# ViTAE-Transformer/LeMeViT

Measured on AMD Instinct MI355X. Metric: images/sec LeMeViT-Base 224^2 bf16 fwd+bwd, higher is better.
Workload: dtype bf16; 1 GPU; lemevit_base 224x224 bf16-autocast train step (fwd+bwd+AdamW), batch 128/GPU, drop_path 0.1, random-init weights; global_batch=128, parallelism=dp1, launch=eager, weight-gradient GEMMs on a side stream

## Files before the change

### lemevit_amd/csrc/attn_mfma.hip

```cpp
#include <stdlib.h>
#include <atomic>
#include "common.h"
#include "attn_internal.h"

#ifndef LMV_XCD_REMAP
#define LMV_XCD_REMAP 1
#endif

namespace {

constexpr int D = 32;
typedef __attribute__((address_space(3))) bf16x4_t* lds4_t;

__device__ __forceinline__ int swz(int r, int c16) { return r * 64 + ((c16 ^ (((r >> 2) & 1) << 1)) << 4); }

template <int NTHREADS>
__device__ __forceinline__ void stage_rows2(unsigned char* sa, const bf16_t* ba, int64_t rsa, unsigned char* sb, const bf16_t* bb, int64_t rsb,
                                            int r0, int nrows, int L, int tid) {
  const int total = nrows * 4, last = max(L - 1, 0);
  for (int c0 = 0; c0 < total; c0 += NTHREADS * 4) {
    uint4 va[4], vb[4];
#pragma unroll
    for (int j = 0; j < 4; ++j) {
      const int c = min(c0 + j * NTHREADS + tid, total - 1), cc = c & 3;
// ... 132 lines not shown
        o0 = MFMA(vt0, ph, o0); o0 = MFMA(vt0, pl, o0);
        o1 = MFMA(vt1, ph, o1); o1 = MFMA(vt1, pl, o1);
      }
    }
    if (q < a.Lq) {
      const float inv = 1.f / l;
      o0 *= inv; o1 *= inv;
      store8(ob + (int64_t)q * a.o_rs, g, o0, o1);
      if (a.lse && g == 0) a.lse[((int64_t)b * a.H + h) * a.Lq + q] = m * a.scale + __logf(l);
    }
  }
}

template <int NKT, int LK = 0, bool PV16 = false>
__global__ __launch_bounds__(256) void mfma_fwd_kernel(const AttnArgs a, int qt_per_block) {
  const int nb = gridDim.x, n = nb * a.H * a.B;
  const int L = LMV_XCD_REMAP ? xcd_contiguous((int)blockIdx.x + nb * ((int)blockIdx.y + a.H * (int)blockIdx.z), n) : (int)blockIdx.x + nb * ((int)blockIdx.y + a.H * (int)blockIdx.z);
  mfma_fwd_body<NKT, LK, PV16>(a, qt_per_block, L % nb, (L / nb) % a.H, L / (nb * a.H));
}

template <int NKT1, int LK1, int NKT2, int LK2>
__global__ __launch_bounds__(256) void mfma_fwd_pair_kernel(const AttnArgs a1, const AttnArgs a2, int per1, int per2, int nblk1) {
  const int n1 = nblk1 * a1.H * a1.B;
  int id = (int)blockIdx.x;
  if (id < n1 && LMV_XCD_REMAP) id = xcd_contiguous(id, n1);
  if (id < n1) { const int bx = id % nblk1, t = id / nblk1; mfma_fwd_body<NKT1, LK1, true>(a1, per1, bx, t % a1.H, t / a1.H); }
  else { const int t = id - n1; mfma_fwd_body<NKT2, LK2, true>(a2, per2, 0, t % a2.H, t / a2.H); }
}

template <int NKT>
__global__ __launch_bounds__(256) void mfma_bwd_dq_kernel(const AttnArgs a, float* __restrict__ delta, int qt_per_block) {
  __shared__ __attribute__((aligned(16))) unsigned char sK[NKT * 16 * 64], sV[NKT * 16 * 64];
  const int tid = threadIdx.x, lane = tid & 63, wave = tid >> 6, h = blockIdx.y, b = blockIdx.z;
  const bf16_t* qb = reinterpret_cast<const bf16_t*>(a.q) + b * a.q_bs + h * D;
  const bf16_t* gb = reinterpret_cast<const bf16_t*>(a.d_o) + b * a.o_bs + h * D;
  const bf16_t* ob = reinterpret_cast<const bf16_t*>(a.o) + b * a.o_bs + h * D;
  bf16_t* dqb = reinterpret_cast<bf16_t*>(a.dq) + b * a.q_bs + h * D;
  stage_rows2<256>(sK, reinterpret_cast<const bf16_t*>(a.k) + b * a.k_bs + h * D, a.k_rs, sV, reinterpret_cast<const bf16_t*>(a.v) + b * a.v_bs + h * D, a.v_rs, 0, NKT * 16, a.Lk, tid);
  __syncthreads();
  const int nqt = (a.Lq + 15) >> 4;
  const int qt_end = min(nqt, (int)(blockIdx.x + 1) * qt_per_block);
  const int g = lane >> 4;
  const int64_t bh = ((int64_t)b * a.H + h) * a.Lq;
  for (int qt = blockIdx.x * qt_per_block + wave; qt < qt_end; qt += 4) {
    const int q = qt * 16 + (lane & 15);
    const bool vq = q < a.Lq;
    const bf16x8_t qf = load_frag_global(qb, a.q_rs, q, a.Lq, lane);
    const bf16x8_t gf = load_frag_global(gb, a.o_rs, q, a.Lq, lane);
    const bf16x8_t of = load_frag_global(ob, a.o_rs, q, a.Lq, lane);
    const float lse = vq ? a.lse[bh + q] : 0.f;
    float dl = 0.f;
#pragma unroll
    for (int j = 0; j < 8; ++j) dl += (float)gf[j] * (float)of[j];
    dl = group_sum4(dl);
    if (vq && g == 0) delta[bh + q] = dl;
    f32x4_t dq0 = {0.f, 0.f, 0.f, 0.f}, dq1 = {0.f, 0.f, 0.f, 0.f};
#pragma unroll
    for (int kb2 = 0; kb2 < NKT / 2; ++kb2) {
      f32x4_t ds[2];
#pragma unroll
      for (int t = 0; t < 2; ++t) {
        const int kt = 2 * kb2 + t;
        const f32x4_t s = MFMA(frag_n(sK, kt * 16, lane), qf, (f32x4_t{0.f, 0.f, 0.f, 0.f}));
        const f32x4_t dp = MFMA(frag_n(sV, kt * 16, lane), gf, (f32x4_t{0.f, 0.f, 0.f, 0.f}));
#pragma unroll
        for (int r = 0; r < 4; ++r) {
          const bool ok = vq && (kt * 16 + g * 4 + r < a.Lk);
          const float p = ok ? __expf(s[r] * a.scale - lse) : 0.f;
          ds[t][r] = p * (dp[r] - dl) * a.scale;
        }
      }
      const bf16x8_t dsf = pack8(ds[0], ds[1]);
      dq0 = MFMA(frag_t(sK, kb2 * 32, kb2 * 32 + 16, 0, lane), dsf, dq0);
      dq1 = MFMA(frag_t(sK, kb2 * 32, kb2 * 32 + 16, 16, lane), dsf, dq1);
    }
    if (vq) {
      store8(dqb + (int64_t)q * a.q_rs, g, dq0, dq1);
    }
  }
}

constexpr int QR_MAX = 448;

template <int NKT, int KW, bool ATOMIC, bool FUSEDQ = false, int LK = 0, int QRM = QR_MAX>
__device__ __forceinline__ void mfma_bwd_dkv_body(const AttnArgs& a, const float* __restrict__ delta, float* __restrict__ acc_k,
                                                  float* __restrict__ acc_v, int q_per_block, const int bx, const int h, const int b) {
  constexpr int QW = 4 / KW;
  constexpr int TPW = (NKT + KW - 1) / KW;
  const int Lk = LK ? LK : a.Lk;
  static_assert(!FUSEDQ || (NKT == 2 && KW == 1), "the fused dQ path is written for two key tiles per wave");
  __shared__ __attribute__((aligned(16))) unsigned char sQG[2 * QRM * 64];
  __shared__ __attribute__((aligned(16))) float sL[QRM], sDl[QRM];
  __shared__ __attribute__((aligned(16))) unsigned char sKV[FUSEDQ ? 2 * 32 * 64 : 16];
  unsigned char* sQ = sQG;
  unsigned char* sG = sQG + QRM * 64;
  const int tid = threadIdx.x, lane = tid & 63, wave = tid >> 6;
  const int kw = wave % KW, qw = wave / KW, g = lane >> 4;
  const int q0 = bx * q_per_block, q1 = min(a.Lq, q0 + q_per_block);
  const int nrows = ((q1 - q0 + 31) >> 5) << 5;
  const int64_t bh = ((int64_t)b * a.H + h) * a.Lq;
  stage_rows2<256>(sQ, reinterpret_cast<const bf16_t*>(a.q) + b * a.q_bs + h * D, a.q_rs, sG, reinterpret_cast<const bf16_t*>(a.d_o) + b * a.o_bs + h * D, a.o_rs, q0, nrows, q1, tid);
  const bf16_t* kb = reinterpret_cast<const bf16_t*>(a.k) + b * a.k_bs + h * D;
  const bf16_t* vb = reinterpret_cast<const bf16_t*>(a.v) + b * a.v_bs + h * D;
  for (int i = tid; i < nrows; i += 256) {
    const bool ok = q0 + i < q1;
    sL[i] = ok ? a.lse[bh + q0 + i] : 1e30f;
    if constexpr (FUSEDQ) {
      float dl = 0.f;
      if (ok) {
        const bf16_t* gp = reinterpret_cast<const bf16_t*>(a.d_o) + b * a.o_bs + (int64_t)(q0 + i) * a.o_rs + h * D;
        const bf16_t* op = reinterpret_cast<const bf16_t*>(a.o) + b * a.o_bs + (int64_t)(q0 + i) * a.o_rs + h * D;
        uint4 rg[4], ro[4];
#pragma unroll
        for (int c = 0; c < 4; ++c) { rg[c] = *reinterpret_cast<const uint4*>(gp + c * 8); ro[c] = *reinterpret_cast<const uint4*>(op + c * 8); }
#pragma unroll
        for (int c = 0; c < 4; ++c) {
          float gv[8], ov[8];
          chunk_to_f<bf16_t>(rg[c], gv); chunk_to_f<bf16_t>(ro[c], ov);
#pragma unroll
          for (int j = 0; j < 8; ++j) dl += gv[j] * ov[j];
        }
      }
      sDl[i] = dl;
    } else {
      sDl[i] = ok ? delta[bh + q0 + i] : 0.f;
    }
  }
  if constexpr (FUSEDQ) stage_rows2<256>(sKV, kb, a.k_rs, sKV + 32 * 64, vb, a.v_rs, 0, 32, Lk, tid);
  bf16x8_t kf[TPW], vf[TPW];
  f32x4_t dk[TPW][2], dv[TPW][2];
#pragma unroll
  for (int i = 0; i < TPW; ++i) {
    const int kt = kw + i * KW;
    kf[i] = load_frag_global(kb, a.k_rs, kt * 16 + (lane & 15), (kt < NKT) ? Lk : 0, lane);
    vf[i] = load_frag_global(vb, a.v_rs, kt * 16 + (lane & 15), (kt < NKT) ? Lk : 0, lane);
#pragma unroll
    for (int dt = 0; dt < 2; ++dt) { dk[i][dt] = f32x4_t{0.f, 0.f, 0.f, 0.f}; dv[i][dt] = f32x4_t{0.f, 0.f, 0.f, 0.f}; }
  }
  __syncthreads();
  const bool vkey = true;
  for (int qb = qw; qb * 32 < nrows; qb += QW) {
    const int r0 = qb * 32;
    const bf16x8_t qn0 = frag_n(sQ, r0, lane), qn1 = frag_n(sQ, r0 + 16, lane);
    const bf16x8_t gn0 = frag_n(sG, r0, lane), gn1 = frag_n(sG, r0 + 16, lane);
    const bf16x8_t qt0 = frag_t(sQ, r0, r0 + 16, 0, lane), qt1 = frag_t(sQ, r0, r0 + 16, 16, lane);
    const bf16x8_t gt0 = frag_t(sG, r0, r0 + 16, 0, lane), gt1 = frag_t(sG, r0, r0 + 16, 16, lane);
    const float4 l0 = *reinterpret_cast<const float4*>(sL + r0 + g * 4), l1 = *reinterpret_cast<const float4*>(sL + r0 + 16 + g * 4);
    const float4 d0 = *reinterpret_cast<const float4*>(sDl + r0 + g * 4), d1 = *reinterpret_cast<const float4*>(sDl + r0 + 16 + g * 4);
    const float lse[8] = {l0.x, l0.y, l0.z, l0.w, l1.x, l1.y, l1.z, l1.w};
    const float dl[8] = {d0.x, d0.y, d0.z, d0.w, d1.x, d1.y, d1.z, d1.w};
    if constexpr (FUSEDQ) {
      bf16_t* dqb = reinterpret_cast<bf16_t*>(a.dq) + b * a.q_bs + h * D;
#pragma unroll
      for (int t = 0; t < 2; ++t) {
        const int qi = r0 + t * 16 + (lane & 15);
        const float lq = sL[qi], dq_ = sDl[qi];
        const bf16x8_t qn = t ? qn1 : qn0, gn = t ? gn1 : gn0;
        f32x4_t dsq[2];
#pragma unroll
        for (int kt = 0; kt < 2; ++kt) {
          if (LK && kt * 16 >= LK) { dsq[kt] = f32x4_t{0.f, 0.f, 0.f, 0.f}; continue; }
          const f32x4_t sv = MFMA(kf[kt], qn, (f32x4_t{0.f, 0.f, 0.f, 0.f}));
          const f32x4_t dp = MFMA(vf[kt], gn, (f32x4_t{0.f, 0.f, 0.f, 0.f}));
#pragma unroll
          for (int r = 0; r < 4; ++r) {
            const bool kin = (LK && kt * 16 + 16 <= LK) ? true : (kt * 16 + g * 4 + r < Lk);
            const float pq = kin ? __expf(sv[r] * a.scale - lq) : 0.f;
            dsq[kt][r] = pq * (dp[r] - dq_) * a.scale;
          }
        }
        const bf16x8_t dsf = pack8(dsq[0], dsq[1]);
// ... 124 lines not shown
    for (int dt = 0; dt < 2; ++dt) { dk[i][dt] = f32x4_t{0.f, 0.f, 0.f, 0.f}; dv[i][dt] = f32x4_t{0.f, 0.f, 0.f, 0.f}; }
  }
  __syncthreads();
  bf16_t* dqb = reinterpret_cast<bf16_t*>(a.dq) + b * a.q_bs + h * D;
  for (int r0 = 0; r0 < nrows; r0 += 32) {
    const bf16x8_t qn0 = frag_n(sQ, r0, lane), qn1 = frag_n(sQ, r0 + 16, lane);
    const bf16x8_t gn0 = frag_n(sG, r0, lane), gn1 = frag_n(sG, r0 + 16, lane);
    const bf16x8_t qt0 = frag_t(sQ, r0, r0 + 16, 0, lane), qt1 = frag_t(sQ, r0, r0 + 16, 16, lane);
    const bf16x8_t gt0 = frag_t(sG, r0, r0 + 16, 0, lane), gt1 = frag_t(sG, r0, r0 + 16, 16, lane);
    const float4 l0 = *reinterpret_cast<const float4*>(sL + r0 + g * 4), l1 = *reinterpret_cast<const float4*>(sL + r0 + 16 + g * 4);
    const float4 d0 = *reinterpret_cast<const float4*>(sDl + r0 + g * 4), d1 = *reinterpret_cast<const float4*>(sDl + r0 + 16 + g * 4);
    const float lse[8] = {l0.x, l0.y, l0.z, l0.w, l1.x, l1.y, l1.z, l1.w};
    const float dl[8] = {d0.x, d0.y, d0.z, d0.w, d1.x, d1.y, d1.z, d1.w};
#pragma unroll
    for (int i = 0; i < TPW; ++i) {
      const int kt = wave + i * 4;
      if (kt >= NKT || kt * 16 >= Lk) continue;
      const bool kvalid = kt * 16 + (lane & 15) < Lk;
      const f32x4_t s0 = MFMA(qn0, kf[i], (f32x4_t{0.f, 0.f, 0.f, 0.f})), s1 = MFMA(qn1, kf[i], (f32x4_t{0.f, 0.f, 0.f, 0.f}));
      const f32x4_t p0 = MFMA(gn0, vf[i], (f32x4_t{0.f, 0.f, 0.f, 0.f})), p1 = MFMA(gn1, vf[i], (f32x4_t{0.f, 0.f, 0.f, 0.f}));
      f32x4_t pr[2], ds[2];
#pragma unroll
      for (int r = 0; r < 4; ++r) {
        const float e0 = kvalid ? __expf(s0[r] * a.scale - lse[r]) : 0.f, e1 = kvalid ? __expf(s1[r] * a.scale - lse[4 + r]) : 0.f;
        pr[0][r] = e0; pr[1][r] = e1;
        ds[0][r] = e0 * (p0[r] - dl[r]) * a.scale; ds[1][r] = e1 * (p1[r] - dl[4 + r]) * a.scale;
      }
      const bf16x8_t pf = pack8(pr[0], pr[1]), dsf = pack8(ds[0], ds[1]);
      dv[i][0] = MFMA(gt0, pf, dv[i][0]); dv[i][1] = MFMA(gt1, pf, dv[i][1]);
      dk[i][0] = MFMA(qt0, dsf, dk[i][0]); dk[i][1] = MFMA(qt1, dsf, dk[i][1]);
      const uint4 w = __builtin_bit_cast(uint4, dsf);
      *reinterpret_cast<uint2*>(sT(wave, 0, i) + (lane & 15) * 32 + g * 8) = make_uint2(w.x, w.y);
      *reinterpret_cast<uint2*>(sT(wave, 1, i) + (lane & 15) * 32 + g * 8) = make_uint2(w.z, w.w);
    }
    f32x4_t dq[2][2];
#pragma unroll
    for (int t = 0; t < 2; ++t) { dq[t][0] = f32x4_t{0.f, 0.f, 0.f, 0.f}; dq[t][1] = f32x4_t{0.f, 0.f, 0.f, 0.f}; }
    {
      const int rr = (lane & 15) >> 2, qq = lane & 3;
#pragma unroll
      for (int pp = 0; pp < NP; ++pp) {
        const int kta = wave + (2 * pp) * 4, ktb = wave + (2 * pp + 1) * 4;
        if (kta >= NKT || kta * 16 >= Lk) continue;
        const bool has_b = 2 * pp + 1 < TPW && ktb < NKT && ktb * 16 < Lk;
        const int rowb = has_b ? ktb * 16 : kta * 16;
        const bf16x8_t ka = frag_t(sK, kta * 16, rowb, 0, lane), kb2 = frag_t(sK, kta * 16, rowb, 16, lane);
#pragma unroll
        for (int t = 0; t < 2; ++t) {
          const bf16x4_t lo = __builtin_amdgcn_ds_read_tr16_b64_v4bf16((lds4_t)(sT(wave, t, 2 * pp) + (g * 4 + rr) * 32 + qq * 8));
          bf16x4_t hi = {(__bf16)0.f, (__bf16)0.f, (__bf16)0.f, (__bf16)0.f};
          if (has_b) hi = __builtin_amdgcn_ds_read_tr16_b64_v4bf16((lds4_t)(sT(wave, t, 2 * pp + (2 * pp + 1 < TPW ? 1 : 0)) + (g * 4 + rr) * 32 + qq * 8));
          const bf16x8_t dst = __builtin_shufflevector(lo, hi, 0, 1, 2, 3, 4, 5, 6, 7);
          dq[t][0] = MFMA(ka, dst, dq[t][0]); dq[t][1] = MFMA(kb2, dst, dq[t][1]);
        }
      }
    }
#pragma unroll
    for (int t = 0; t < 2; ++t)
#pragma unroll
      for (int hh = 0; hh < 2; ++hh) *reinterpret_cast<f32x4_t*>(sRed(wave, t * 2 + hh) + lane * 4) = dq[t][hh];
    __syncthreads();
    if (wave < 2) {
      f32x4_t x0 = {0.f, 0.f, 0.f, 0.f}, x1 = {0.f, 0.f, 0.f, 0.f};
#pragma unroll
      for (int w = 0; w < 4; ++w) {
        x0 += *reinterpret_cast<const f32x4_t*>(sRed(w, wave * 2) + lane * 4);
        x1 += *reinterpret_cast<const f32x4_t*>(sRed(w, wave * 2 + 1) + lane * 4);
      }
      const int q = r0 + wave * 16 + (lane & 15);
      if (q < Lq) store8(dqb + (int64_t)q * a.q_rs, g, x0, x1);
    }
    __syncthreads();
  }
#pragma unroll
  for (int i = 0; i < TPW; ++i) {
    const int kt = wave + i * 4, key = kt * 16 + (lane & 15);
    if (kt >= NKT || key >= Lk) continue;
    store8(reinterpret_cast<bf16_t*>(a.dk) + b * a.k_bs + (int64_t)key * a.k_rs + h * D, g, dk[i][0], dk[i][1]);
    store8(reinterpret_cast<bf16_t*>(a.dv) + b * a.v_bs + (int64_t)key * a.v_rs + h * D, g, dv[i][0], dv[i][1]);
  }
}


template <int NKT, int LK = 0>
__device__ __forceinline__ void mfma_bwd_fused_body2(const AttnArgs& a, const int h, const int b) {
  constexpr int TPW = (NKT + 3) / 4;
  constexpr int NPAIR = (NKT + 1) / 2;
  constexpr int NQ = NKT * 16;
  constexpr int TBUF = 4 * 2 * TPW * 512;
  __shared__ __attribute__((aligned(16))) unsigned char sQ[NQ * 64], sG[NQ * 64];
  __shared__ __attribute__((aligned(16))) unsigned char sKT[(2 * TBUF > NQ * 64) ? 2 * TBUF : NQ * 64];
  __shared__ __attribute__((aligned(16))) float sL[NQ], sDl[NQ];
  auto sT = [&](int buf, int w, int t, int slot) -> unsigned char* { return &sKT[buf * TBUF + ((w * 2 + t) * TPW + slot) * 512]; };
  const int tid = threadIdx.x, lane = tid & 63, wave = __builtin_amdgcn_readfirstlane(tid >> 6);
  const int g = lane >> 4;
  const int Lk = LK ? LK : a.Lk, Lq = a.Lq;
  const int nrows = ((Lq + 31) >> 5) << 5;
  const int64_t bh = ((int64_t)b * a.H + h) * Lq;
  const bf16_t* kb = reinterpret_cast<const bf16_t*>(a.k) + b * a.k_bs + h * D;
  const bf16_t* vb = reinterpret_cast<const bf16_t*>(a.v) + b * a.v_bs + h * D;
  stage_rows2<256>(sQ, reinterpret_cast<const bf16_t*>(a.q) + b * a.q_bs + h * D, a.q_rs, sG, reinterpret_cast<const bf16_t*>(a.d_o) + b * a.o_bs + h * D, a.o_rs, 0, nrows, Lq, tid);
  stage_rows2<256>(sKT, kb, a.k_rs, sKT, kb, a.k_rs, 0, NKT * 16, Lk, tid);
  for (int i = tid; i < nrows; i += 256) {
    const bool ok = i < Lq;
    sL[i] = ok ? a.lse[bh + i] : 1e30f;
    float dl = 0.f;
    if (ok) {
      const bf16_t* gp = reinterpret_cast<const bf16_t*>(a.d_o) + b * a.o_bs + (int64_t)i * a.o_rs + h * D;
      const bf16_t* op = reinterpret_cast<const bf16_t*>(a.o) + b * a.o_bs + (int64_t)i * a.o_rs + h * D;
      uint4 rg[4], ro[4];
#pragma unroll
      for (int c = 0; c < 4; ++c) { rg[c] = *reinterpret_cast<const uint4*>(gp + c * 8); ro[c] = *reinterpret_cast<const uint4*>(op + c * 8); }
#pragma unroll
      for (int c = 0; c < 4; ++c) {
        float gv[8], ov[8];
        chunk_to_f<bf16_t>(rg[c], gv); chunk_to_f<bf16_t>(ro[c], ov);
#pragma unroll
        for (int j = 0; j < 8; ++j) dl += gv[j] * ov[j];
      }
    }
    sDl[i] = dl;
  }
  bf16x8_t kf[TPW], vf[TPW];
  f32x4_t dk[TPW][2], dv[TPW][2];
#pragma unroll
  for (int i = 0; i < TPW; ++i) {
    const int kt = wave + i * 4;
    kf[i] = load_frag_global(kb, a.k_rs, kt * 16 + (lane & 15), (kt < NKT) ? Lk : 0, lane);
    vf[i] = load_frag_global(vb, a.v_rs, kt * 16 + (lane & 15), (kt < NKT) ? Lk : 0, lane);
#pragma unroll
    for (int dt = 0; dt < 2; ++dt) { dk[i][dt] = f32x4_t{0.f, 0.f, 0.f, 0.f}; dv[i][dt] = f32x4_t{0.f, 0.f, 0.f, 0.f}; }
  }
  __syncthreads();
  const int qt_w = wave >> 1, dh = wave & 1;
  bf16x8_t ktf[NPAIR];
#pragma unroll
  for (int pp = 0; pp < NPAIR; ++pp) {
    const int rowb = (2 * pp + 1 < NKT) ? (2 * pp + 1) * 16 : 2 * pp * 16;
    ktf[pp] = frag_t(sKT, 2 * pp * 16, rowb, dh * 16, lane);
  }
  __syncthreads();
  bf16_t* dqb = reinterpret_cast<bf16_t*>(a.dq) + b * a.q_bs + h * D;
  int buf = 0;
  for (int r0 = 0; r0 < nrows; r0 += 32, buf ^= 1) {
    const bf16x8_t qn0 = frag_n(sQ, r0, lane), qn1 = frag_n(sQ, r0 + 16, lane);
    const bf16x8_t gn0 = frag_n(sG, r0, lane), gn1 = frag_n(sG, r0 + 16, lane);
    const bf16x8_t qt0 = frag_t(sQ, r0, r0 + 16, 0, lane), qt1 = frag_t(sQ, r0, r0 + 16, 16, lane);
    const bf16x8_t gt0 = frag_t(sG, r0, r0 + 16, 0, lane), gt1 = frag_t(sG, r0, r0 + 16, 16, lane);
    const float4 l0 = *reinterpret_cast<const float4*>(sL + r0 + g * 4), l1 = *reinterpret_cast<const float4*>(sL + r0 + 16 + g * 4);
    const float4 d0 = *reinterpret_cast<const float4*>(sDl + r0 + g * 4), d1 = *reinterpret_cast<const float4*>(sDl + r0 + 16 + g * 4);
    const float lse[8] = {l0.x, l0.y, l0.z, l0.w, l1.x, l1.y, l1.z, l1.w};
    const float dl[8] = {d0.x, d0.y, d0.z, d0.w, d1.x, d1.y, d1.z, d1.w};
#pragma unroll
    for (int i = 0; i < TPW; ++i) {
      const int kt = wave + i * 4;
      if (kt >= NKT || kt * 16 >= Lk) continue;
      const bool kvalid = kt * 16 + (lane & 15) < Lk;
      const f32x4_t s0 = MFMA(qn0, kf[i], (f32x4_t{0.f, 0.f, 0.f, 0.f})), s1 = MFMA(qn1, kf[i], (f32x4_t{0.f, 0.f, 0.f, 0.f}));
      const f32x4_t p0 = MFMA(gn0, vf[i], (f32x4_t{0.f, 0.f, 0.f, 0.f})), p1 = MFMA(gn1, vf[i], (f32x4_t{0.f, 0.f, 0.f, 0.f}));
      f32x4_t pr[2], ds[2];
#pragma unroll
      for (int r = 0; r < 4; ++r) {
        const float e0 = kvalid ? __expf(s0[r] * a.scale - lse[r]) : 0.f, e1 = kvalid ? __expf(s1[r] * a.scale - lse[4 + r]) : 0.f;
        pr[0][r] = e0; pr[1][r] = e1;
        ds[0][r] = e0 * (p0[r] - dl[r]) * a.scale; ds[1][r] = e1 * (p1[r] - dl[4 + r]) * a.scale;
      }
      const bf16x8_t pf = pack8(pr[0], pr[1]), dsf = pack8(ds[0], ds[1]);
      dv[i][0] = MFMA(gt0, pf, dv[i][0]); dv[i][1] = MFMA(gt1, pf, dv[i][1]);
      dk[i][0] = MFMA(qt0, dsf, dk[i][0]); dk[i][1] = MFMA(qt1, dsf, dk[i][1]);
      const uint4 w = __builtin_bit_cast(uint4, dsf);
      const int wsl = (g ^ ((lane >> 2) & 3)) * 8;
      *reinterpret_cast<uint2*>(sT(buf, wave, 0, i) + (lane & 15) * 32 + wsl) = make_uint2(w.x, w.y);
      *reinterpret_cast<uint2*>(sT(buf, wave, 1, i) + (lane & 15) * 32 + wsl) = make_uint2(w.z, w.w);
    }
    __syncthreads();
    {
      const int rr = (lane & 15) >> 2, qq = lane & 3;
      f32x4_t dq = {0.f, 0.f, 0.f, 0.f};
#pragma unroll
      for (int pp = 0; pp < NPAIR; ++pp) {
        const int kta = 2 * pp, ktb = 2 * pp + 1;
        if (kta * 16 >= Lk) continue;
        const bool has_b = ktb < NKT && ktb * 16 < Lk;
        const bf16x4_t lo = __builtin_amdgcn_ds_read_tr16_b64_v4bf16((lds4_t)(sT(buf, kta & 3, qt_w, kta >> 2) + (g * 4 + rr) * 32 + (qq ^ g) * 8));
        bf16x4_t hi = {(__bf16)0.f, (__bf16)0.f, (__bf16)0.f, (__bf16)0.f};
        if (has_b) hi = __builtin_amdgcn_ds_read_tr16_b64_v4bf16((lds4_t)(sT(buf, ktb & 3, qt_w, ktb >> 2) + (g * 4 + rr) * 32 + (qq ^ g) * 8));
        const bf16x8_t dst = __builtin_shufflevector(lo, hi, 0, 1, 2, 3, 4, 5, 6, 7);
        dq = MFMA(ktf[pp], dst, dq);
      }
      const int q = r0 + qt_w * 16 + (lane & 15);
      if (q < Lq) store4(dqb + (int64_t)q * a.q_rs + g * 8 + dh * 4, dq);
    }
  }
#pragma unroll
  for (int i = 0; i < TPW; ++i) {
    const int kt = wave + i * 4, key = kt * 16 + (lane & 15);
    if (kt >= NKT || key >= Lk) continue;
    store8(reinterpret_cast<bf16_t*>(a.dk) + b * a.k_bs + (int64_t)key * a.k_rs + h * D, g, dk[i][0], dk[i][1]);
    store8(reinterpret_cast<bf16_t*>(a.dv) + b * a.v_bs + (int64_t)key * a.v_rs + h * D, g, dv[i][0], dv[i][1]);
  }
}

template <int NKT, int LK = 0, int VER = 1>
__global__ __launch_bounds__(256, 2) void mfma_bwd_fused_kernel(const AttnArgs a) {
  const int n = a.H * a.B, id = (int)blockIdx.y + a.H * (int)blockIdx.z;
  const int L = LMV_XCD_REMAP ? xcd_contiguous(id, n) : id;
  if constexpr (VER == 2) mfma_bwd_fused_body2<NKT, LK>(a, L % a.H, L / a.H);
  else mfma_bwd_fused_body<NKT, LK>(a, L % a.H, L / a.H);
}

template <int NKT1, int LK1, int VER = 1>
__global__ __launch_bounds__(256, 2) void mfma_bwd_pair_kernel(const AttnArgs a1, const AttnArgs a2) {
  const int n1 = a1.H * a1.B;
  int id = (int)blockIdx.x;
  if (id < n1 && LMV_XCD_REMAP) id = xcd_contiguous(id, n1);
  if (id < n1) { if constexpr (VER == 2) mfma_bwd_fused_body2<NKT1, LK1>(a1, id % a1.H, id / a1.H); else mfma_bwd_fused_body<NKT1, LK1>(a1, id % a1.H, id / a1.H); }
  else mfma_bwd_dkv_body<2, 1, false, true, 16, 32>(a2, nullptr, nullptr, nullptr, 32, 0, (id - n1) % a2.H, (id - n1) / a2.H);
}

__global__ __launch_bounds__(256) void scatter_bf16_kernel(const float* __restrict__ acc, bf16_t* __restrict__ dst, int64_t bs, int64_t rs, int B, int H,
                                                          int L, int LP) {
  const unsigned idx = blockIdx.x * 256 + threadIdx.x, total = (unsigned)B * H * L * D;
  if (idx >= total) return;
  const unsigned d = idx % D, l = (idx / D) % L, h = (idx / (D * L)) % H, b = idx / (D * L * H);
  dst[b * bs + (int64_t)l * rs + h * D + d] = f2bf(acc[((((int64_t)b * H + h) * LP) + l) * D + d]);
}

__global__ __launch_bounds__(256) void scatter_sum_kernel(const float* __restrict__ acc0, const float* __restrict__ acc1, bf16_t* __restrict__ dst0,
                                                         bf16_t* __restrict__ dst1, int64_t bs0, int64_t rs0, int64_t bs1, int64_t rs1, int B, int H, int L,
                                                         int LP, int nslab) {
  const unsigned idx = blockIdx.x * 256 + threadIdx.x, per = (unsigned)B * H * L * (D / 4);
  if (idx >= 2 * per) return;
  const bool second = idx >= per;
  const unsigned i = second ? idx - per : idx;
  const unsigned d4 = i % (D / 4), l = (i / (D / 4)) % L, h = (i / ((D / 4) * L)) % H, b = i / ((D / 4) * L * H);
  const float* src = (second ? acc1 : acc0) + ((((int64_t)b * H + h) * LP) + l) * D + d4 * 4;
  const int64_t slab = (int64_t)B * H * LP * D;
  f32x4_t s = {0.f, 0.f, 0.f, 0.f};
  for (int k = 0; k < nslab; ++k) s += *reinterpret_cast<const f32x4_t*>(src + k * slab);
  bf16_t* dst = second ? dst1 + b * bs1 + (int64_t)l * rs1 + h * D + d4 * 4 : dst0 + b * bs0 + (int64_t)l * rs0 + h * D + d4 * 4;
  store4(dst, s);
}

constexpr int RKT = 8, RK = RKT * 16;
constexpr int RKT_B = 4, RKB = RKT_B * 16;

__global__ __launch_bounds__(256) void mfma_fwd_split_kernel(const AttnArgs a, float* __restrict__ part, int nsplit) {
  __shared__ __attribute__((aligned(16))) unsigned char sK[4 * RK * 64], sV[4 * RK * 64];
  const int tid = threadIdx.x, lane = tid & 63, wave = tid >> 6, g = lane >> 4;
  const int nbx = gridDim.x, Lid = LMV_XCD_REMAP ? xcd_contiguous((int)blockIdx.x + nbx * ((int)blockIdx.y + a.H * (int)blockIdx.z), nbx * a.H * a.B)
                                                 : (int)blockIdx.x + nbx * ((int)blockIdx.y + a.H * (int)blockIdx.z);
  const int bx = Lid % nbx, h = (Lid / nbx) % a.H, b = Lid / (nbx * a.H);
  const int split = bx * 4 + wave, k0 = split * RK;
  const bf16_t* kb = reinterpret_cast<const bf16_t*>(a.k) + b * a.k_bs + h * D;
  const bf16_t* vb = reinterpret_cast<const bf16_t*>(a.v) + b * a.v_bs + h * D;
  unsigned char* wK = sK + wave * RK * 64;
  unsigned char* wV = sV + wave * RK * 64;
  stage_rows2<64>(wK, kb, a.k_rs, wV, vb, a.v_rs, k0, RK, a.Lk, lane);
  asm volatile("s_waitcnt vmcnt(0) lgkmcnt(0)" ::: "memory");
  __builtin_amdgcn_wave_barrier();
  if (split >= nsplit) return;
  const int q = lane & 15;
  float* pp = part + ((((int64_t)b * a.H + h) * nsplit + split) * 16 + q) * (D + 2);
  if (k0 >= a.Lk) {
    if (g == 0) { pp[0] = -1e30f; pp[1] = 0.f; }
#pragma unroll
    for (int r = 0; r < 4; ++r) { pp[2 + g * 4 + r] = 0.f; pp[18 + g * 4 + r] = 0.f; }
    return;
  }
  const bf16x8_t qf = load_frag_global(reinterpret_cast<const bf16_t*>(a.q) + b * a.q_bs + h * D, a.q_rs, q, a.Lq, lane);
  f32x4_t s[RKT];
  float m = -1e30f;
#pragma unroll
  for (int kt = 0; kt < RKT; ++kt) {
    s[kt] = MFMA(frag_n(wK, kt * 16, lane), qf, (f32x4_t{0.f, 0.f, 0.f, 0.f}));
#pragma unroll
    for (int r = 0; r < 4; ++r) {
      s[kt][r] = (k0 + kt * 16 + g * 4 + r < a.Lk) ? s[kt][r] * a.scale : -1e30f;
      m = fmaxf(m, s[kt][r]);
    }
  }
  m = group_max4(m);
  float l = 0.f;
#pragma unroll
  for (int kt = 0; kt < RKT; ++kt)
#pragma unroll
    for (int r = 0; r < 4; ++r) { const float p = __expf(s[kt][r] - m); s[kt][r] = p; l += p; }
  l = group_sum4(l);
  f32x4_t o0 = {0.f, 0.f, 0.f, 0.f}, o1 = {0.f, 0.f, 0.f, 0.f};
#pragma unroll
  for (int kb2 = 0; kb2 < RKT / 2; ++kb2) {
    const bf16x8_t ph = pack8(s[2 * kb2], s[2 * kb2 + 1]);
    f32x4_t r0, r1;
#pragma unroll
    for (int r = 0; r < 4; ++r) { r0[r] = s[2 * kb2][r] - (float)ph[r]; r1[r] = s[2 * kb2 + 1][r] - (float)ph[4 + r]; }
    const bf16x8_t pl = pack8(r0, r1);
    const bf16x8_t vt0 = frag_t(wV, kb2 * 32, kb2 * 32 + 16, 0, lane), vt1 = frag_t(wV, kb2 * 32, kb2 * 32 + 16, 16, lane);
    o0 = MFMA(vt0, ph, o0); o0 = MFMA(vt0, pl, o0);
    o1 = MFMA(vt1, ph, o1); o1 = MFMA(vt1, pl, o1);
  }
// ... 580 lines not shown
  dkv_split(a, &nsplit, &qpb);
  return 2 * (size_t)nsplit * a.B * a.H * nkt_for(a.Lk) * 16 * D * sizeof(float);
}

int lmv_attn_mfma_fwd(const AttnArgs& a, hipStream_t st) {
  const int per = qt_per_block_for(a), nqt = (a.Lq + 15) / 16;
  dim3 grid((nqt + per - 1) / per, a.H, a.B), block(256);
  if (a.Lk == 196) hipLaunchKernelGGL((mfma_fwd_kernel<14, 196, true>), grid, block, 0, st, a, per);
  else if (a.Lk == 16) hipLaunchKernelGGL((mfma_fwd_kernel<2, 16, true>), grid, block, 0, st, a, per);
  else if (a.Lk == 49) hipLaunchKernelGGL((mfma_fwd_kernel<4, 49, true>), grid, block, 0, st, a, per);
  else
  switch (nkt_for(a.Lk)) {
    case 2: hipLaunchKernelGGL((mfma_fwd_kernel<2>), grid, block, 0, st, a, per); break;
    case 4: hipLaunchKernelGGL((mfma_fwd_kernel<4>), grid, block, 0, st, a, per); break;
    case 8: hipLaunchKernelGGL((mfma_fwd_kernel<8>), grid, block, 0, st, a, per); break;
    default: hipLaunchKernelGGL((mfma_fwd_kernel<14>), grid, block, 0, st, a, per); break;
  }
  LMV_CHECK_LAUNCH("attn_mfma_fwd");
  return LMV_OK;
}

int lmv_attn_mfma_bwd(const AttnArgs& a, float* delta, float* acc, hipStream_t st) {
  const int per = qt_per_block_for(a), nqt = (a.Lq + 15) / 16, nkt = nkt_for(a.Lk);
  if (nkt >= 4 && a.Lq > 16 && a.Lq <= nkt * 16) {
    dim3 grid(1, a.H, a.B), block(256);
    if (a.Lk == 196) hipLaunchKernelGGL((mfma_bwd_fused_kernel<14, 196, 2>), grid, block, 0, st, a);
    else if (a.Lk == 49) hipLaunchKernelGGL((mfma_bwd_fused_kernel<4, 49, 2>), grid, block, 0, st, a);
    else if (nkt == 4) hipLaunchKernelGGL((mfma_bwd_fused_kernel<4>), grid, block, 0, st, a);
    else if (nkt == 8) hipLaunchKernelGGL((mfma_bwd_fused_kernel<8>), grid, block, 0, st, a);
    else hipLaunchKernelGGL((mfma_bwd_fused_kernel<14>), grid, block, 0, st, a);
    LMV_CHECK_LAUNCH("attn_mfma_bwd_fused");
    return LMV_OK;
  }
  if (nkt == 14 && a.Lq > 16) {
    int nk, pr, lds;
    if (int rc = long_geometry(a, &nk, &pr, &lds)) return rc;
    hipLaunchKernelGGL(mfma_bwd_dq_long_kernel, dim3((nqt + pr - 1) / pr, a.H, a.B), dim3(256), lds, st, a, delta, pr, nk);
  } else if (nkt != 2) {
    dim3 grid((nqt + per - 1) / per, a.H, a.B), block(256);
    switch (nkt) {
      case 4: hipLaunchKernelGGL((mfma_bwd_dq_kernel<4>), grid, block, 0, st, a, delta, per); break;
      case 8: hipLaunchKernelGGL((mfma_bwd_dq_kernel<8>), grid, block, 0, st, a, delta, per); break;
      default: hipLaunchKernelGGL((mfma_bwd_dq_kernel<14>), grid, block, 0, st, a, delta, per); break;
    }
  }
  int nsplit, qpb;
  dkv_split(a, &nsplit, &qpb);
  dim3 grid(nsplit, a.H, a.B), block(256);
  const size_t acc_elems = (size_t)nsplit * a.B * a.H * nkt * 16 * D;
  float* acc_k = acc; float* acc_v = acc + acc_elems;
  if (nsplit > 1) {
#define DKV(N, K) hipLaunchKernelGGL((mfma_bwd_dkv_kernel<N, K, true>), grid, block, 0, st, a, delta, acc_k, acc_v, qpb)
    if (nkt == 2 && a.Lk == 16) hipLaunchKernelGGL((mfma_bwd_dkv_kernel<2, 1, true, true, 16>), grid, block, 0, st, a, delta, acc_k, acc_v, qpb);
    else if (nkt == 2) hipLaunchKernelGGL((mfma_bwd_dkv_kernel<2, 1, true, true>), grid, block, 0, st, a, delta, acc_k, acc_v, qpb);
    else
    switch (nkt) { case 4: DKV(4, 2); break; case 8: DKV(8, 4); break; default: DKV(14, 4); break; }
#undef DKV
    const unsigned n = 2u * (unsigned)a.B * a.H * a.Lk * (D / 4);
    hipLaunchKernelGGL(scatter_sum_kernel, dim3((n + 255) / 256), dim3(256), 0, st, (const float*)acc_k, (const float*)acc_v, (bf16_t*)a.dk, (bf16_t*)a.dv,
                       a.k_bs, a.k_rs, a.v_bs, a.v_rs, a.B, a.H, a.Lk, nkt * 16, nsplit);
  } else {
#define DKV(N, K) hipLaunchKernelGGL((mfma_bwd_dkv_kernel<N, K, false>), grid, block, 0, st, a, delta, acc_k, acc_v, qpb)
    if (nkt == 2 && a.Lk == 16) hipLaunchKernelGGL((mfma_bwd_dkv_kernel<2, 1, false, true, 16>), grid, block, 0, st, a, delta, acc_k, acc_v, qpb);
    else if (nkt == 2) hipLaunchKernelGGL((mfma_bwd_dkv_kernel<2, 1, false, true>), grid, block, 0, st, a, delta, acc_k, acc_v, qpb);
    else
    switch (nkt) { case 4: DKV(4, 2); break; case 8: DKV(8, 4); break; default: DKV(14, 4); break; }
#undef DKV
  }
  LMV_CHECK_LAUNCH("attn_mfma_bwd");
  return LMV_OK;
}

int lmv_attn_mfma_fwd_pair(const AttnArgs& a1, const AttnArgs& a2, hipStream_t st) {
  if (a1.B != a2.B || a1.H != a2.H || a2.Lk != 16 || a2.Lq != 16 || a1.Lq != a1.Lk || (a1.Lk != 196 && a1.Lk != 49)) return 0;
  const int per1 = qt_per_block_for(a1), nqt1 = (a1.Lq + 15) / 16, nblk1 = (nqt1 + per1 - 1) / per1;
  dim3 grid((nblk1 + 1) * a1.H * a1.B), block(256);
  if (a1.Lk == 196) hipLaunchKernelGGL((mfma_fwd_pair_kernel<14, 196, 2, 16>), grid, block, 0, st, a1, a2, per1, 1, nblk1);
  else hipLaunchKernelGGL((mfma_fwd_pair_kernel<4, 49, 2, 16>), grid, block, 0, st, a1, a2, per1, 1, nblk1);
  return 1;
}

int lmv_attn_mfma_bwd_pair(const AttnArgs& a1, const AttnArgs& a2, hipStream_t st) {
  if (a1.B != a2.B || a1.H != a2.H || a2.Lk != 16 || a2.Lq != 16 || a1.Lq != a1.Lk || (a1.Lk != 196 && a1.Lk != 49)) return 0;
  dim3 grid(2 * a1.H * a1.B), block(256);
  if (a1.Lk == 196) hipLaunchKernelGGL((mfma_bwd_pair_kernel<14, 196, 2>), grid, block, 0, st, a1, a2);
  else hipLaunchKernelGGL((mfma_bwd_pair_kernel<4, 49, 2>), grid, block, 0, st, a1, a2);
  return 1;
}
```

Measured before the change: 4278 images/sec.

## Use 8-wave fused attention backward for 196 tokens and per-image meta-token blocks

Result: no change. 4258 images/sec (median of 2 runs) (-0.5%).

```diff
diff --git a/lemevit_amd/csrc/attn_mfma.hip b/lemevit_amd/csrc/attn_mfma.hip
--- a/lemevit_amd/csrc/attn_mfma.hip
+++ b/lemevit_amd/csrc/attn_mfma.hip
@@ -238,11 +238,12 @@
 
 constexpr int QR_MAX = 448;
 
-template <int NKT, int KW, bool ATOMIC, bool FUSEDQ = false, int LK = 0, int QRM = QR_MAX>
+template <int NKT, int KW, bool ATOMIC, bool FUSEDQ = false, int LK = 0>
 __device__ __forceinline__ void mfma_bwd_dkv_body(const AttnArgs& a, const float* __restrict__ delta, float* __restrict__ acc_k,
                                                   float* __restrict__ acc_v, int q_per_block, const int bx, const int h, const int b) {
   constexpr int QW = 4 / KW;
   constexpr int TPW = (NKT + KW - 1) / KW;
+  constexpr int QRM = QR_MAX;
   const int Lk = LK ? LK : a.Lk;
   static_assert(!FUSEDQ || (NKT == 2 && KW == 1), "the fused dQ path is written for two key tiles per wave");
   __shared__ __attribute__((aligned(16))) unsigned char sQG[2 * QRM * 64];
@@ -533,16 +534,24 @@
 }
 
 
+template <int NKT>
+constexpr int bwd_body2_lds() {
+  constexpr int TBUF = 4 * 2 * ((NKT + 3) / 4) * 512, NQ = NKT * 16;
+  return 2 * NQ * 64 + ((2 * TBUF > NQ * 64) ? 2 * TBUF : NQ * 64) + 2 * NQ * 4;
+}
 template <int NKT, int LK = 0>
-__device__ __forceinline__ void mfma_bwd_fused_body2(const AttnArgs& a, const int h, const int b) {
+__device__ __forceinline__ void mfma_bwd_fused_body2(const AttnArgs& a, const int h, const int b, unsigned char* smem) {
   constexpr int TPW = (NKT + 3) / 4;
   constexpr int NPAIR = (NKT + 1) / 2;
   constexpr int NQ = NKT * 16;
   constexpr int TBUF = 4 * 2 * TPW * 512;
-  __shared__ __attribute__((aligned(16))) unsigned char sQ[NQ * 64], sG[NQ * 64];
-  __shared__ __attribute__((aligned(16))) unsigned char sKT[(2 * TBUF > NQ * 64) ? 2 * TBUF : NQ * 64];
-  __shared__ __attribute__((aligned(16))) float sL[NQ], sDl[NQ];
-  auto sT = [&](int buf, int w, int t, int slot) -> unsigned char* { return &sKT[buf * TBUF + ((w * 2 + t) * TPW + slot) * 512]; };
+  constexpr int KTSZ = (2 * TBUF > NQ * 64) ? 2 * TBUF : NQ * 64;
+  unsigned char* sQ = smem;
+  unsigned char* sG = smem + NQ * 64;
+  unsigned char* sKT = smem + 2 * NQ * 64;
+  float* sL = reinterpret_cast<float*>(sKT + KTSZ);
+  float* sDl = sL + NQ;
+  auto sT = [&](int buf, int w, int t, int slot) -> unsigned char* { return sKT + buf * TBUF + ((w * 2 + t) * TPW + slot) * 512; };
   const int tid = threadIdx.x, lane = tid & 63, wave = __builtin_amdgcn_readfirstlane(tid >> 6);
   const int g = lane >> 4;
   const int Lk = LK ? LK : a.Lk, Lq = a.Lq;
@@ -652,21 +661,236 @@
   }
 }
 
+template <int NKT>
+constexpr int bwd_body3_lds() { return 3 * NKT * 16 * 64 + 2 * (16 * 2 * 512) + 2 * NKT * 16 * 4; }
+template <int NKT, int LK>
+__device__ __forceinline__ void mfma_bwd_fused_body3(const AttnArgs& a, const int h, const int b, unsigned char* smem) {
+  constexpr int NW = 8, NT = NW * 64, TPW = 2;
+  constexpr int NPAIR = (NKT + 1) / 2;
+  constexpr int NQ = NKT * 16;
+  constexpr int TBUF = NW * TPW * 2 * 512;
+  static_assert(LK > 0 && NKT > NW && NKT <= NW * TPW && (NKT & 1) == 0, "written for 9 .. 16 key tiles with a compile-time key count");
+  unsigned char* sQ = smem;
+  unsigned char* sG = smem + NQ * 64;
+  unsigned char* sK = smem + 2 * NQ * 64;
+  unsigned char* sTB = smem + 3 * NQ * 64;
+  float* sL = reinterpret_cast<float*>(sTB + 2 * TBUF);
+  float* sDl = sL + NQ;
+  auto sT = [&](int buf, int kt, int t) -> unsigned char* { return sTB + buf * TBUF + (kt * 2 + t) * 512; };
+  const int tid = threadIdx.x, lane = tid & 63, wave = __builtin_amdgcn_readfirstlane(tid >> 6);
+  const int g = lane >> 4;
+  constexpr int Lk = LK;
+  const int Lq = a.Lq;
+  const int nrows = ((Lq + 31) >> 5) << 5;
+  const int64_t bh = ((int64_t)b * a.H + h) * Lq;
+  const bf16_t* kb = reinterpret_cast<const bf16_t*>(a.k) + b * a.k_bs + h * D;
+  const bf16_t* vb = reinterpret_cast<const bf16_t*>(a.v) + b * a.v_bs + h * D;
+  stage_rows2<NT>(sQ, reinterpret_cast<const bf16_t*>(a.q) + b * a.q_bs + h * D, a.q_rs, sG, reinterpret_cast<const bf16_t*>(a.d_o) + b * a.o_bs + h * D, a.o_rs, 0, nrows, Lq, tid);
+  stage_rows2<NT>(sK, kb, a.k_rs, sK, kb, a.k_rs, 0, NKT * 16, Lk, tid);
+  for (int i = tid; i < nrows; i += NT) {
+    const bool ok = i < Lq;
+    sL[i] = ok ? a.lse[bh + i] : 1e30f;
+    float dl = 0.f;
+    if (ok) {
+      const bf16_t* gp = reinterpret_cast<const bf16_t*>(a.d_o) + b * a.o_bs + (int64_t)i * a.o_rs + h * D;
+      const bf16_t* op = reinterpret_cast<const bf16_t*>(a.o) + b * a.o_bs + (int64_t)i * a.o_rs + h * D;
+      uint4 rg[4], ro[4];
+#pragma unroll
+      for (int c = 0; c < 4; ++c) { rg[c] = *reinterpret_cast<const uint4*>(gp + c * 8); ro[c] = *reinterpret_cast<const uint4*>(op + c * 8); }
+#pragma unroll
+      for (int c = 0; c < 4; ++c) {
+        float gv[8], ov[8];
+        chunk_to_f<bf16_t>(rg[c], gv); chunk_to_f<bf16_t>(ro[c], ov);
+#pragma unroll
+        for (int j = 0; j < 8; ++j) dl += gv[j] * ov[j];
+      }
+    }
+    sDl[i] = dl;
+  }
+  bf16x8_t kf[TPW], vf[TPW];
+  f32x4_t dk[TPW][2], dv[TPW][2];
+#pragma unroll
+  for (int i = 0; i < TPW; ++i) {
+    const int kt = wave + i * NW;
+    kf[i] = load_frag_global(kb, a.k_rs, kt * 16 + (lane & 15), (kt < NKT) ? Lk : 0, lane);
+    vf[i] = load_frag_global(vb, a.v_rs, kt * 16 + (lane & 15), (kt < NKT) ? Lk : 0, lane);
+#pragma unroll
+    for (int dt = 0; dt < 2; ++dt) { dk[i][dt] = f32x4_t{0.f, 0.f, 0.f, 0.f}; dv[i][dt] = f32x4_t{0.f, 0.f, 0.f, 0.f}; }
+  }
+  __syncthreads();
+  bf16_t* dqb = reinterpret_cast<bf16_t*>(a.dq) + b * a.q_bs + h * D;
+  int buf = 0;
+  for (int r0 = 0; r0 < nrows; r0 += 32, buf ^= 1) {
+    {
+        const float4 l0 = *reinterpret_cast<const float4*>(sL + r0 + g * 4), l1 = *reinterpret_cast<const float4*>(sL + r0 + 16 + g * 4);
+        const float4 d0 = *reinterpret_cast<const float4*>(sDl + r0 + g * 4), d1 = *reinterpret_cast<const float4*>(sDl + r0 + 16 + g * 4);
+        const float lse[8] = {l0.x, l0.y, l0.z, l0.w, l1.x, l1.y, l1.z, l1.w};
+        const float dl[8] = {d0.x, d0.y, d0.z, d0.w, d1.x, d1.y, d1.z, d1.w};
+#pragma unroll
+      for (int i = 0; i < TPW; ++i) {
+        const int kt = wave + i * NW;
+        if (kt >= NKT || kt * 16 >= Lk) continue;
+        const bf16x8_t qn0 = frag_n(sQ, r0, lane), qn1 = frag_n(sQ, r0 + 16, lane);
+        const bf16x8_t gn0 = frag_n(sG, r0, lane), gn1 = frag_n(sG, r0 + 16, lane);
+        const bool kvalid = kt * 16 + (lane & 15) < Lk;
+        const f32x4_t s0 = MFMA(qn0, kf[i], (f32x4_t{0.f, 0.f, 0.f, 0.f})), s1 = MFMA(qn1, kf[i], (f32x4_t{0.f, 0.f, 0.f, 0.f}));
+        const f32x4_t p0 = MFMA(gn0, vf[i], (f32x4_t{0.f, 0.f, 0.f, 0.f})), p1 = MFMA(gn1, vf[i], (f32x4_t{0.f, 0.f, 0.f, 0.f}));
+        f32x4_t pr[2], ds[2];
+#pragma unroll
+        for (int r = 0; r < 4; ++r) {
+          const float e0 = kvalid ? __expf(s0[r] * a.scale - lse[r]) : 0.f, e1 = kvalid ? __expf(s1[r] * a.scale - lse[4 + r]) : 0.f;
+          pr[0][r] = e0; pr[1][r] = e1;
+          ds[0][r] = e0 * (p0[r] - dl[r]) * a.scale; ds[1][r] = e1 * (p1[r] - dl[4 + r]) * a.scale;
+        }
+        const bf16x8_t pf = pack8(pr[0], pr[1]), dsf = pack8(ds[0], ds[1]);
+        dv[i][0] = MFMA(frag_t(sG, r0, r0 + 16, 0, lane), pf, dv[i][0]); dv[i][1] = MFMA(frag_t(sG, r0, r0 + 16, 16, lane), pf, dv[i][1]);
+        dk[i][0] = MFMA(frag_t(sQ, r0, r0 + 16, 0, lane), dsf, dk[i][0]); dk[i][1] = MFMA(frag_t(sQ, r0, r0 + 16, 16, lane), dsf, dk[i][1]);
+        const uint4 w = __builtin_bit_cast(uint4, dsf);
+        const int wsl = (g ^ ((lane >> 2) & 3)) * 8;
+        *reinterpret_cast<uint2*>(sT(buf, kt, 0) + (lane & 15) * 32 + wsl) = make_uint2(w.x, w.y);
+        *reinterpret_cast<uint2*>(sT(buf, kt, 1) + (lane & 15) * 32 + wsl) = make_uint2(w.z, w.w);
+      }
+    }
+    __syncthreads();
+    if (wave >= NW - 4) {
+      const int qt_w = (wave - (NW - 4)) >> 1, dh = wave & 1;
+      const int rr = (lane & 15) >> 2, qq = lane & 3;
+      f32x4_t dq = {0.f, 0.f, 0.f, 0.f};
+#pragma unroll
+      for (int pp = 0; pp < NPAIR; ++pp) {
+        const int kta = 2 * pp, ktb = 2 * pp + 1;
+        if (kta * 16 >= Lk) continue;
+        const bool has_b = ktb * 16 < Lk;
+        const bf16x4_t lo = __builtin_amdgcn_ds_read_tr16_b64_v4bf16((lds4_t)(sT(buf, kta, qt_w) + (g * 4 + rr) * 32 + (qq ^ g) * 8));
+        bf16x4_t hi = {(__bf16)0.f, (__bf16)0.f, (__bf16)0.f, (__bf16)0.f};
+        if (has_b) hi = __builtin_amdgcn_ds_read_tr16_b64_v4bf16((lds4_t)(sT(buf, ktb, qt_w) + (g * 4 + rr) * 32 + (qq ^ g) * 8));
+        const bf16x8_t dst = __builtin_shufflevector(lo, hi, 0, 1, 2, 3, 4, 5, 6, 7);
+        dq = MFMA(frag_t(sK, kta * 16, ktb * 16, dh * 16, lane), dst, dq);
+      }
+      const int q = r0 + qt_w * 16 + (lane & 15);
+      if (q < Lq) store4(dqb + (int64_t)q * a.q_rs + g * 8 + dh * 4, dq);
+    }
+  }
+#pragma unroll
+  for (int i = 0; i < TPW; ++i) {
+    const int kt = wave + i * NW, key = kt * 16 + (lane & 15);
+    if (kt >= NKT || key >= Lk) continue;
+    store8(reinterpret_cast<bf16_t*>(a.dk) + b * a.k_bs + (int64_t)key * a.k_rs + h * D, g, dk[i][0], dk[i][1]);
+    store8(reinterpret_cast<bf16_t*>(a.dv) + b * a.v_bs + (int64_t)key * a.v_rs + h * D, g, dv[i][0], dv[i][1]);
+  }
+}
+
 template <int NKT, int LK = 0, int VER = 1>
 __global__ __launch_bounds__(256, 2) void mfma_bwd_fused_kernel(const AttnArgs a) {
   const int n = a.H * a.B, id = (int)blockIdx.y + a.H * (int)blockIdx.z;
   const int L = LMV_XCD_REMAP ? xcd_contiguous(id, n) : id;
-  if constexpr (VER == 2) mfma_bwd_fused_body2<NKT, LK>(a, L % a.H, L / a.H);
-  else mfma_bwd_fused_body<NKT, LK>(a, L % a.H, L / a.H);
-}
-
-template <int NKT1, int LK1, int VER = 1>
-__global__ __launch_bounds__(256, 2) void mfma_bwd_pair_kernel(const AttnArgs a1, const AttnArgs a2) {
+  if constexpr (VER == 2) {
+    __shared__ __attribute__((aligned(16))) unsigned char smem[bwd_body2_lds<NKT>()];
+    mfma_bwd_fused_body2<NKT, LK>(a, L % a.H, L / a.H, smem);
+  } else mfma_bwd_fused_body<NKT, LK>(a, L % a.H, L / a.H);
+}
+
+constexpr int META_LDS = 3 * 16 * 64 + 2 * 16 * 4;
+__device__ __forceinline__ bf16x8_t frag_t16(const unsigned char* s, int d0, int lane) {
+  const int g = lane >> 4, i = lane & 15;
+  const bf16x4_t lo = __builtin_amdgcn_ds_read_tr16_b64_v4bf16((lds4_t)(s + swz(g * 4 + (i >> 2), i & 3) + (d0 >> 4) * 8));
+  const bf16x4_t hi = {(__bf16)0.f, (__bf16)0.f, (__bf16)0.f, (__bf16)0.f};
+  return __builtin_shufflevector(lo, hi, 0, 1, 2, 3, 4, 5, 6, 7);
+}
+template <int NW>
+__device__ __forceinline__ void meta_bwd_image(const AttnArgs& a, const int b, unsigned char* smem) {
+  const int lane = threadIdx.x & 63, wave = __builtin_amdgcn_readfirstlane((int)threadIdx.x >> 6);
+  const int g = lane >> 4, c = lane & 15;
+  unsigned char* sQ = smem + wave * META_LDS;
+  unsigned char* sG = sQ + 16 * 64;
+  unsigned char* sK = sG + 16 * 64;
+  float* sL = reinterpret_cast<float*>(sK + 16 * 64);
+  float* sDl = sL + 16;
+  const f32x4_t z = {0.f, 0.f, 0.f, 0.f};
+  for (int h0 = 0; h0 < a.H; h0 += NW) {
+    const int h = h0 + wave;
+    const bool active = h < a.H;
+    const bf16_t* qb = reinterpret_cast<const bf16_t*>(a.q) + b * a.q_bs + h * D;
+    const bf16_t* kb = reinterpret_cast<const bf16_t*>(a.k) + b * a.k_bs + h * D;
+    const bf16_t* vb = reinterpret_cast<const bf16_t*>(a.v) + b * a.v_bs + h * D;
+    const bf16_t* gb = reinterpret_cast<const bf16_t*>(a.d_o) + b * a.o_bs + h * D;
+    const bf16_t* ob = reinterpret_cast<const bf16_t*>(a.o) + b * a.o_bs + h * D;
+    bf16x8_t kf = {}, vf = {};
+    if (h0) __syncthreads();
+    if (active) {
+      const int r = lane >> 2, cc = lane & 3;
+      const uint4 cq = *reinterpret_cast<const uint4*>(qb + (int64_t)r * a.q_rs + cc * 8);
+      const uint4 cg = *reinterpret_cast<const uint4*>(gb + (int64_t)r * a.o_rs + cc * 8);
+      const uint4 ck = *reinterpret_cast<const uint4*>(kb + (int64_t)r * a.k_rs + cc * 8);
+      kf = load_frag_global(kb, a.k_rs, c, 16, lane);
+      vf = load_frag_global(vb, a.v_rs, c, 16, lane);
+      *reinterpret_cast<uint4*>(sQ + swz(r, cc)) = cq;
+      *reinterpret_cast<uint4*>(sG + swz(r, cc)) = cg;
+      *reinterpret_cast<uint4*>(sK + swz(r, cc)) = ck;
+      if (lane < 16) {
+        sL[lane] = a.lse[((int64_t)b * a.H + h) * 16 + lane];
+        float dl = 0.f;
+        const bf16_t* gp = gb + (int64_t)lane * a.o_rs;
+        const bf16_t* op = ob + (int64_t)lane * a.o_rs;
+        uint4 rg[4], ro[4];
+#pragma unroll
+        for (int j = 0; j < 4; ++j) { rg[j] = *reinterpret_cast<const uint4*>(gp + j * 8); ro[j] = *reinterpret_cast<const uint4*>(op + j * 8); }
+#pragma unroll
+        for (int j = 0; j < 4; ++j) {
+          float gv[8], ov[8];
+          chunk_to_f<bf16_t>(rg[j], gv); chunk_to_f<bf16_t>(ro[j], ov);
+#pragma unroll
+          for (int e = 0; e < 8; ++e) dl += gv[e] * ov[e];
+        }
+        sDl[lane] = dl;
+      }
+    }
+    __syncthreads();
+    if (active) {
+      const bf16x8_t qn = frag_n(sQ, 0, lane), gn = frag_n(sG, 0, lane);
+      {
+        const float lq = sL[c], dq_ = sDl[c];
+        const f32x4_t sv = MFMA(kf, qn, z), dp = MFMA(vf, gn, z);
+        f32x4_t dsq;
+#pragma unroll
+        for (int r = 0; r < 4; ++r) dsq[r] = __expf(sv[r] * a.scale - lq) * (dp[r] - dq_) * a.scale;
+        const bf16x8_t dsf = pack8(dsq, z);
+        const f32x4_t dq0 = MFMA(frag_t16(sK, 0, lane), dsf, z), dq1 = MFMA(frag_t16(sK, 16, lane), dsf, z);
+        store8(reinterpret_cast<bf16_t*>(a.dq) + b * a.q_bs + (int64_t)c * a.q_rs + h * D, g, dq0, dq1);
+      }
+      {
+        const float4 l0 = *reinterpret_cast<const float4*>(sL + g * 4), d0 = *reinterpret_cast<const float4*>(sDl + g * 4);
+        const float lse[4] = {l0.x, l0.y, l0.z, l0.w}, dl[4] = {d0.x, d0.y, d0.z, d0.w};
+        const f32x4_t s0 = MFMA(qn, kf, z), p0 = MFMA(gn, vf, z);
+        f32x4_t pr, ds;
+#pragma unroll
+        for (int r = 0; r < 4; ++r) {
+          const float e0 = __expf(s0[r] * a.scale - lse[r]);
+          pr[r] = e0;
+          ds[r] = e0 * (p0[r] - dl[r]) * a.scale;
+        }
+        const bf16x8_t pf = pack8(pr, z), dsf = pack8(ds, z);
+        const f32x4_t dv0 = MFMA(frag_t16(sG, 0, lane), pf, z), dv1 = MFMA(frag_t16(sG, 16, lane), pf, z);
+        const f32x4_t dk0 = MFMA(frag_t16(sQ, 0, lane), dsf, z), dk1 = MFMA(frag_t16(sQ, 16, lane), dsf, z);
+        store8(reinterpret_cast<bf16_t*>(a.dk) + b * a.k_bs + (int64_t)c * a.k_rs + h * D, g, dk0, dk1);
+        store8(reinterpret_cast<bf16_t*>(a.dv) + b * a.v_bs + (int64_t)c * a.v_rs + h * D, g, dv0, dv1);
+      }
+    }
+  }
+}
+
+template <int NKT1, int LK1, int VER>
+__global__ __launch_bounds__(VER == 3 ? 512 : 256, VER == 3 ? 4 : 2) void mfma_bwd_pair_kernel(const AttnArgs a1, const AttnArgs a2) {
+  constexpr int NW = VER == 3 ? 8 : 4;
+  constexpr int IMG = VER == 3 ? bwd_body3_lds<NKT1>() : bwd_body2_lds<NKT1>();
+  __shared__ __attribute__((aligned(16))) unsigned char smem[IMG > NW * META_LDS ? IMG : NW * META_LDS];
   const int n1 = a1.H * a1.B;
   int id = (int)blockIdx.x;
   if (id < n1 && LMV_XCD_REMAP) id = xcd_contiguous(id, n1);
-  if (id < n1) { if constexpr (VER == 2) mfma_bwd_fused_body2<NKT1, LK1>(a1, id % a1.H, id / a1.H); else mfma_bwd_fused_body<NKT1, LK1>(a1, id % a1.H, id / a1.H); }
-  else mfma_bwd_dkv_body<2, 1, false, true, 16, 32>(a2, nullptr, nullptr, nullptr, 32, 0, (id - n1) % a2.H, (id - n1) / a2.H);
+  if (id < n1) {
+    if constexpr (VER == 3) mfma_bwd_fused_body3<NKT1, LK1>(a1, id % a1.H, id / a1.H, smem);
+    else mfma_bwd_fused_body2<NKT1, LK1>(a1, id % a1.H, id / a1.H, smem);
+  } else meta_bwd_image<NW>(a2, id - n1, smem);
 }
 
 __global__ __launch_bounds__(256) void scatter_bf16_kernel(const float* __restrict__ acc, bf16_t* __restrict__ dst, int64_t bs, int64_t rs, int B, int H,
@@ -1413,8 +1637,8 @@
 
 int lmv_attn_mfma_bwd_pair(const AttnArgs& a1, const AttnArgs& a2, hipStream_t st) {
   if (a1.B != a2.B || a1.H != a2.H || a2.Lk != 16 || a2.Lq != 16 || a1.Lq != a1.Lk || (a1.Lk != 196 && a1.Lk != 49)) return 0;
-  dim3 grid(2 * a1.H * a1.B), block(256);
-  if (a1.Lk == 196) hipLaunchKernelGGL((mfma_bwd_pair_kernel<14, 196, 2>), grid, block, 0, st, a1, a2);
-  else hipLaunchKernelGGL((mfma_bwd_pair_kernel<4, 49, 2>), grid, block, 0, st, a1, a2);
+  dim3 grid(a1.H * a1.B + a1.B);
+  if (a1.Lk == 196) hipLaunchKernelGGL((mfma_bwd_pair_kernel<14, 196, 3>), grid, dim3(512), 0, st, a1, a2);
+  else hipLaunchKernelGGL((mfma_bwd_pair_kernel<4, 49, 2>), grid, dim3(256), 0, st, a1, a2);
   return 1;
 }
```
